# cvxgrp/cvxpygen

Hardware: AMD Instinct MI355X
Metric: QP instances solved/sec (batched MPC QP, OSQP; inputs resident in HBM) (higher is better)
Workload: dtype f64

## Files before the change

### cvxpygen_amd/codegen.py

```python

from __future__ import annotations

import os
import shutil
import subprocess
from typing import List, Optional, Sequence

import numpy as np

from .solve_program import GEN_EXTRA_SLOTS, LANES, RaggedProgram, execution_steps, padded_offsets_fit

CSRC = os.path.join(os.path.dirname(os.path.abspath(__file__)), 'csrc')


class ProgramTooLarge(Exception):
    """the family's solve program cannot be made LDS-resident: no specialised library for it"""


def emit_program_header(rp: RaggedProgram, name: str = 'family', plan=None, depth: int = 2, cross: int = 4,
                        pad_offsets: bool = False, group_offsets: int = 4, batch: int = 1, early: int = 4) -> str:
    out: List[str] = []
    w = out.append
    w(f'// Generated by cvxpygen_amd.codegen for problem family "{name}" -- do not edit.')
    w(f'// solve program: {rp.n_phases} phases, {rp.n_chunks} chunks, {int(rp.ctab[:, 0].sum())} steps, '
# ... 537 lines not shown
    if sync:
        for _ in plist:
            w('        cpgw::block_sync();')
    w('    } break;')
    w('    }')
    w('}')
    w('}  // namespace cpg')
    return '\n'.join(out) + '\n' + epilogue


def factor_fingerprint(fac) -> int:
    h = 0x811C9DC5
    ct = np.asarray(fac.ctab, dtype=np.int32).reshape(-1, 4)[:, [0, 1, 3]]
    for arr in (np.ascontiguousarray(ct), np.ascontiguousarray(fac.tlen, dtype=np.uint32)):
        for b in arr.tobytes():
            h = ((h ^ b) * 0x01000193) & 0xFFFFFFFF
    return h


FACTOR_LOOKAHEAD = int(os.environ.get('CPG_FACTOR_LOOKAHEAD', 3))
FACTOR_BY_LEVEL = os.environ.get('CPG_FACTOR_BY_LEVEL', '1') != '0'
FACTOR_LOOKAHEAD_CHUNKS = int(os.environ.get('CPG_FACTOR_LOOKAHEAD_CHUNKS', 3))
FACTOR_DUMMY_DOUBLES = 2


def factor_levels(ctab) -> List[List[int]]:
    ct = np.asarray(ctab, dtype=np.int64).reshape(-1, 4)
    levels, cur = [], []
    for c in range(ct.shape[0]):
        cur.append(c)
        if int(ct[c, 1]) & 1:
            levels.append(cur)
            cur = []
    if cur:
        levels.append(cur)
    return levels


def factor_chunk_kinds(fac, nnzL: int, N: int, inverse_from: Optional[int] = None) -> List[str]:
    ct = np.asarray(fac.ctab, dtype=np.int64).reshape(-1, 4)
    nch = ct.shape[0]
    task = np.asarray(fac.task, dtype=np.int64).reshape(nch, -1)
    inv0 = nch if inverse_from is None else int(inverse_from)
    kinds = []
    for c in range(nch):
        t = task[c][task[c] != 0xFFFFFFFF] & 0x7FFFFFFF
# ... 307 lines not shown
        return False
    per_wave = max(per_wave, fac + (fac & 1))
    return tab + 8 * 8 * per_wave <= LDS_BYTES


def instance_header(plan, out_dir: str, name: str = 'family') -> Optional[str]:
    from . import refactor_plan as _rp
    d = plan.desc
    o = plan.osqp_shared or plan.osqp
    Ps, As = o.pruned(d.P, d.A)
    rpl = _rp.shared_mode_plan(Ps, As, o)
    if not instance_program_fits(rpl):
        return None
    dims = dict(N=d.n_var, M=d.m, NEQ=d.n_eq)
    mg = rpl.merged
    if mg is None:
        prog, fac = rpl.sol, emit_factor_program(rpl.fac, rpl.nnzL, rpl.n + rpl.m, by_level=FACTOR_BY_LEVEL)
    else:
        import types
        dims['NNZX'] = mg.nnzX
        prog = mg.sol
        fac = emit_factor_program(types.SimpleNamespace(ctab=mg.f_ctab, tlen=mg.f_len, task=mg.f_task), rpl.nnzL, rpl.n + rpl.m,
                                  zero=mg.fac_len - 1, one=mg.one_pos, inverse_from=mg.base.fac.n_chunks, by_level=FACTOR_BY_LEVEL)
    return write_instance_header(prog, os.path.join(os.path.abspath(out_dir), f'cpg_instance_{name}.h'), name,
                                 row_programs=shared_row_programs(Ps, As), dims=dims, epilogue=fac, lean=True)


RESIDENT_MAX_REGS = int(os.environ.get('CPG_RESIDENT_MAX_REGS', 160))
RESIDENT_MAX_STEPS = int(os.environ.get('CPG_RESIDENT_MAX_STEPS', 320))
RESIDENT_ACC_BASE = int(os.environ.get('CPG_RESIDENT_ACC_BASE', 32))
RESIDENT_GATHER_BATCH = int(os.environ.get('CPG_RESIDENT_GATHER_BATCH', 12))
RESIDENT_ACC_PAIRS = int(os.environ.get('CPG_RESIDENT_ACC_PAIRS', 112))


def resident_compiler_flags(defs: Sequence[str]) -> List[str]:
    return []


def matrix_parameters(desc) -> bool:
    import scipy.sparse as _sps
    NP = desc.NP
    return any(_sps.csr_matrix(desc.maps[k])[:, :NP].nnz > 0 for k in ('P', 'A'))


def resident_program_fits(rpl, np_var: Optional[int] = None) -> bool:
    rp = rpl.sol
# ... 716 lines not shown
```

### cvxpygen_amd/csrc/cpg_hip.cpp

```cpp
#include "../../include/cpg_hip.h"

#include <math.h>
#include <stdio.h>
#include <stdlib.h>
#include <string.h>

#include <algorithm>
#include <string>
#include <type_traits>
#include <vector>

#include "cpg_osqp_kernel.h"
#include "cpg_osqp_refactor.h"
#include "cpg_osqp_resident.h"
#include "cpg_osqp_team.h"
#include "cpg_osqp_squad.h"
#include "cpg_clarabel_kernel.h"

#include <hip/hip_runtime.h>
typedef hipStream_t rt_stream_t;
typedef hipEvent_t rt_event_t;
#define RT_CHECK(expr)                                                                         \
    do {                                                                                       \
        hipError_t e_ = (expr);                                                                \
// ... 12 lines not shown
};
struct ResultBufs {
    DevBuf prim, dual, obj, pri, dua, iter, status;
    int ensure(size_t B, const cpg::DevFamily &F);
    void free();
    int copy_out(rt_stream_t stream, size_t first, size_t B, const cpg::DevFamily &F, double *prim_h, double *dual_h,
                 double *obj_h, double *pri_h, double *dua_h, int32_t *iter_h, int32_t *status_h) const;
};

struct cpg_solver_s {
    int device = 0;
    rt_stream_t stream{};
    rt_event_t ev0{}, ev1{};
    bool have_events = false;
    float last_ms = 0.f;
    std::vector<void *> owned;
    std::vector<void *> update_owned;
    cpg::DevFamily F{};
    cpg::DevUpdate U{};
    bool have_update = false;
    cpg::DevRefactor R{};
    bool refactor_mode = false;
    std::vector<void *> refactor_owned;
    cpg::DevResident Rs{};
    std::vector<void *> resident_owned;
    cpg::DevGradient Gd{};
    bool have_gradient = false;
    std::vector<void *> gradient_owned;
    DevBuf g_theta, g_x, g_y, g_dprim, g_dtheta;
    const int *gv_ptr = nullptr, *gv_src = nullptr;
    int n_gv = 0;
    std::vector<void *> gv_owned;
    rt_event_t ev_after{};
    cpg::DevSettings S{};
    int waves_per_block = 0, inst_per_wave = 1, blocks_per_cu = 0;
    int program_in_lds = -1;
    bool squad_ok = false;
    cpg::DevShRegs SRg{};
    bool sreg_ok = false;
    double sreg_rho = 0.0, sreg_sigma = 0.0;
    std::vector<void *> sreg_owned;
    std::vector<void *> ireg_owned;
    int num_cu = 256;
    size_t lds_limit = 160 * 1024;
    unsigned *d_counter = nullptr;
    int n_vary_x = 0, n_vary_z = 0;
// ... 1429 lines not shown
        else if (kind == CPG_K_SIGMA) fkc[d] = h->F.sigma;
        else if (kind == CPG_K_RHO) { if (idx < 0 || (size_t)idx >= m) return false; fkrow[d] = idx; }
        else if (kind != CPG_K_NONE) return false;
    }
    return true;
}

#ifdef CPG_GENI_HEADER
struct InstanceTables {
    int nnzX;
    int sol_chunks, sol_nnz, sol_slots;
    const int32_t *sol_ctab; const uint32_t *sol_desc; const uint16_t *sol_cols; const int32_t *sol_kind, *sol_idx;
    int fac_chunks, fac_triples;
    const int32_t *fac_ctab; const uint32_t *fac_task, *fac_len, *fac_a, *fac_b, *fac_k;
};

static int set_instance_executor(cpg_handle_t h, const cpg_osqp_refactor_t *r, const InstanceTables &g,
                                 const std::vector<double> &fkc, const std::vector<int> &fkrow) {
    std::vector<void *> &own = h->refactor_owned;
    cpg::DevRefactor &R = h->R;
    const size_t n = h->F.n, m = h->F.m, N = n + m;
    int rc = CPG_OK;
    R.gi_ok = 0;
    std::vector<unsigned short> gcols, grows, glcol;
    std::vector<unsigned> gsrc, gdk;
    std::vector<unsigned long long> gtri;
    std::vector<double> gkc;
#ifdef CPG_GENI_N
    const bool geni_dims = h->F.n == CPG_GENI_N && h->F.m == CPG_GENI_M && h->F.n_eq == CPG_GENI_NEQ;
#else
    const bool geni_dims = true;
#endif
#ifdef CPG_GENI_NNZX
    const bool merged_lib = true;
#else
    const bool merged_lib = false;
#endif
    if (!(geni_dims && (g.nnzX > 0) == merged_lib && g.sol_chunks == CPG_GENI_NCHUNKS && g.sol_nnz == CPG_GENI_NNZ && g.sol_slots == CPG_GENI_NSLOTS))
        return CPG_OK;
    const size_t nd = (size_t)r->nnzL + N, nx = (size_t)g.nnzX;
    const unsigned hsh = program_fingerprint(g.sol_ctab, g.sol_desc, g.sol_cols, g.sol_chunks, g.sol_nnz);
    static const int steps[][4] = CPG_GENI_STEPS;
    static const int chunk_shift[] = CPG_GENI_CHUNK_SHIFT;
    bool ok = hsh == CPG_GENI_FINGERPRINT;
    {
        const int nn[3] = {CPG_GENI_AROWS_N, CPG_GENI_PROWS_N, CPG_GENI_ATROWS_N};
        for (int k = 0; ok && k < 3; k++) {
            if ((int)h->rows_hdr[k].size() != 4 * nn[k]) ok = false;
// ... 7 lines not shown
        glcol.assign((size_t)CPG_GENI_NREGS * 64, (unsigned short)0);
        std::vector<char> taken((size_t)CPG_GENI_NREGS * 64, 0);
        for (int t = 0; ok && t < CPG_GENI_NSTEPS; t++) {
            const int e = steps[t][0], cnt = steps[t][1], reg = steps[t][2], sh = steps[t][3];
            if (reg < 0 || reg >= CPG_GENI_NREGS) { ok = false; break; }
            for (int l = 0; l < cnt; l++) {
                int kind = g.sol_kind[e + l], idx = g.sol_idx[e + l];
                if (kind == 4) {
                    if (idx < 0 || (size_t)idx >= nx) { ok = false; break; }
                    kind = 3; idx += (int)N;
                }
                if (kind < 0 || kind > 3 || idx < 0 || idx >= (1 << 28)) { ok = false; break; }
                const size_t at = (size_t)reg * 64 + (size_t)(l + sh);
                if (taken[at]) { ok = false; break; }
                taken[at] = 1;
                gsrc[at] = ((unsigned)kind << 28) | (unsigned)idx;
                if (kind == 2) {
                    if (idx >= r->nnzL || r->Lcol[idx] < 0 || r->Lcol[idx] > 0xFFFF) { ok = false; break; }
                    glcol[at] = (unsigned short)r->Lcol[idx];
                }
            }
        }
    }
#ifdef CPG_GENI_FAC_NSTEPS
    if (ok) {
        static const int fch[][3] = CPG_GENI_FAC_CHUNKS;
        const size_t fac_end = nx ? nd + nx + 2 : nd + 1;
        const size_t one = nd + nx;
        unsigned hsh2 = 0x811C9DC5u;
        auto mix = [&](unsigned v) { for (int k = 0; k < 4; k++) { hsh2 = (hsh2 ^ ((v >> (8 * k)) & 0xFFu)) * 0x01000193u; } };
        const unsigned idle_dst = CPG_GENI_FAC_DUMMY_DOUBLES ? (unsigned)fac_end : 0xFFFFu;
        ok = g.fac_chunks == CPG_GENI_FAC_NCHUNKS && fac_end - 1 == (size_t)CPG_GENI_FAC_ZERO && fac_end + CPG_GENI_FAC_DUMMY_DOUBLES <= 0xFFFFu;
#ifdef CPG_GENI_FAC_ONE
        ok = ok && one == (size_t)CPG_GENI_FAC_ONE;
#endif
        for (int c = 0; ok && c < g.fac_chunks; c++) { mix((unsigned)g.fac_ctab[4 * c]); mix((unsigned)g.fac_ctab[4 * c + 1]); mix((unsigned)g.fac_ctab[4 * c + 3]); }
        for (size_t e = 0; ok && e < (size_t)g.fac_chunks * 64; e++) mix(g.fac_len[e]);
        ok = ok && hsh2 == CPG_GENI_FAC_FINGERPRINT;
        if (ok) {
            const unsigned long long Z = (unsigned long long)(fac_end - 1);
            gtri.assign((size_t)CPG_GENI_FAC_NSTEPS * 64, Z | (Z << 16) | (Z << 32));
            gdk.assign((size_t)g.fac_chunks * 64, idle_dst);
            gkc.assign((size_t)g.fac_chunks * 64, 0.0);
            size_t step = 0;
            for (int c = 0; ok && c < g.fac_chunks; c++) {
                const int L = g.fac_ctab[4 * c];
// ... 22 lines not shown
                    const unsigned t = nx ? (t0 & 0x7FFFFFFFu) : t0;
                    if (t >= nd + nx) { ok = false; break; }
                    const int kr = t < nd ? fkrow[t] : -1;
                    gdk[(size_t)c * 64 + l] = t | ((unsigned)(kr + 1) << 16);
                    gkc[(size_t)c * 64 + l] = t < nd ? fkc[t] : 0.0;
                }
            }
            if (ok && step != (size_t)CPG_GENI_FAC_NSTEPS) ok = false;
        }
        if (ok) {
            if ((rc = upload<unsigned long long>(h, own, gtri.data(), gtri.size(), &R.gf_tri))) return rc;
            if ((rc = upload<unsigned>(h, own, gdk.data(), gdk.size(), &R.gf_dk))) return rc;
            if ((rc = upload<double>(h, own, gkc.data(), gkc.size(), &R.gf_kc))) return rc;
        }
    }
#else
    ok = ok && !nx;
#endif
    if (ok) {
        if ((rc = upload<unsigned short>(h, own, glcol.data(), glcol.size(), &R.gi_lcol))) return rc;
        if ((rc = upload<unsigned short>(h, own, gcols.data(), gcols.size(), &R.gi_cols))) return rc;
        if ((rc = upload<unsigned short>(h, own, grows.data(), grows.size(), &R.gi_rows))) return rc;
        if ((rc = upload<unsigned>(h, own, gsrc.data(), gsrc.size(), &R.gi_src))) return rc;
    }
    if ((rc = rt_sync(h))) return rc;
    R.gi_ok = ok ? 1 : 0;
    return CPG_OK;
}
#endif

int cpg_hip_set_refactor(cpg_handle_t h, const cpg_osqp_refactor_t *r) {
    if (h && h->conic) { set_error("not available for a conic (interior-point) handle"); return CPG_E_BADARG; }
    if (!h || !r) { set_error("null argument"); return CPG_E_BADARG; }
    int rc = rt_set_device(h->device);
    if (rc) return rc;
    if ((rc = rt_sync_linked(h))) return rc;
    free_list(h->refactor_owned);
    free_list(h->resident_owned); h->Rs = cpg::DevResident{};
    free_list(h->ireg_owned);
    std::vector<void *> &own = h->refactor_owned;
    cpg::DevRefactor &R = h->R;
    R.fam_cf = nullptr; R.fam_ct = nullptr; R.fam_rho = 0.0; R.fam_sigma = 0.0;
    const size_t n = h->F.n, m = h->F.m, N = n + m;
    R.nnzP = r->nnzP; R.nnzA = r->nnzA; R.nnzL = r->nnzL; R.n_eq = h->F.n_eq; R.np_var = r->np_var;
    R.scaling_iters = r->scaling_iters; R.d_base = r->d_base;
    R.fac_chunks = r->fac_chunks; R.sol_nnz = r->sol_nnz; R.sol_slots = r->sol_slots;
// ... 49 lines not shown
    if ((rc = upload_csr(h, own, r->map_q, &R.map_q))) return rc;
    if ((rc = upload_csr(h, own, r->map_u, &R.map_u))) return rc;
    if ((rc = upload_csr(h, own, r->map_d, &R.map_d))) return rc;
    R.buf_doubles = (long long)(r->nnzP + 2 * r->nnzA + 3 * n + 4 * m + r->nnzL + 2 * N + std::max(R.sol_nnz, R.gs_nnz) + 64);
    R.shared_mats = r->shared_mats ? 1 : 0; R.cs = 1.0;
    R.Ps = R.As = R.Ars = R.Ds = R.Dinvs = R.Es = R.Einvs = nullptr;
    std::vector<double> ars, dinv, einv;
    if (r->shared_mats) {
        if (!r->Ps || !r->As || !r->D || !r->E || !(r->c > 0.0)) { set_error("shared-matrix mode needs Ps, As, D, E, c"); return CPG_E_BADARG; }
        ars.resize((size_t)r->nnzA); dinv.resize(n); einv.resize(m);
        for (int k = 0; k < r->nnzA; k++) ars[k] = r->As[r->Aent[k]];
        for (size_t i = 0; i < n; i++) dinv[i] = 1.0 / r->D[i];
        for (size_t i = 0; i < m; i++) einv[i] = 1.0 / r->E[i];
        R.cs = r->c;
        if ((rc = upload<double>(h, own, r->Ps, (size_t)r->nnzP, &R.Ps))) return rc;
        if ((rc = upload<double>(h, own, r->As, (size_t)r->nnzA, &R.As))) return rc;
        if ((rc = upload<double>(h, own, ars.data(), ars.size(), &R.Ars))) return rc;
        if ((rc = upload<double>(h, own, r->D, n, &R.Ds))) return rc;
        if ((rc = upload<double>(h, own, dinv.data(), n, &R.Dinvs))) return rc;
        if ((rc = upload<double>(h, own, r->E, m, &R.Es))) return rc;
        if ((rc = upload<double>(h, own, einv.data(), m, &R.Einvs))) return rc;
    }
    R.gf_tri = nullptr; R.gf_dk = nullptr; R.gf_kc = nullptr;
    R.gi_ok = 0; R.gi_cols = R.gi_rows = nullptr; R.gi_src = nullptr; R.gi_lcol = nullptr; R.fac_kc = nullptr; R.fac_krow = nullptr; R.fac_kc_cl = nullptr; R.fac_krow_cl = nullptr; R.fac_kind_cl = nullptr; R.fac_idx_cl = nullptr;
    std::vector<double> fkc, fkc_cl;
    std::vector<int> fkrow, fkrow_cl;

    if (r->shared_mats) {
        if (!kkt_constants(h, r, fkc, fkrow)) { set_error("cpg_hip_set_refactor: KKT source table out of range"); return CPG_E_BADARG; }
        const size_t nd = (size_t)r->nnzL + N;
        fkc_cl.assign((size_t)r->fac_chunks * 64, 0.0); fkrow_cl.assign((size_t)r->fac_chunks * 64, -1);
        for (size_t e = 0; e < fkc_cl.size(); e++) {
            const unsigned t = r->fac_task[e];
            if (t == 0xFFFFFFFFu) continue;
            if (t >= nd) { set_error("cpg_hip_set_refactor: factorisation task out of range"); return CPG_E_BADARG; }
            fkc_cl[e] = fkc[t]; fkrow_cl[e] = fkrow[t];
        }
        if ((rc = upload<double>(h, own, fkc.data(), fkc.size(), &R.fac_kc))) return rc;
        if ((rc = upload<int>(h, own, fkrow.data(), fkrow.size(), &R.fac_krow))) return rc;
        if ((rc = upload<double>(h, own, fkc_cl.data(), fkc_cl.size(), &R.fac_kc_cl))) return rc;
        if ((rc = upload<int>(h, own, fkrow_cl.data(), fkrow_cl.size(), &R.fac_krow_cl))) return rc;
    }
#ifdef CPG_GENI_HEADER
    if (r->shared_mats) {
        const InstanceTables g{0, r->sol_chunks, r->sol_nnz, r->sol_slots, r->sol_ctab, r->sol_desc, r->sol_cols, r->sol_kind, r->sol_idx,
                               r->fac_chunks, r->fac_triples, r->fac_ctab, r->fac_task, r->fac_len, r->fac_a, r->fac_b, r->fac_k};
        if ((rc = set_instance_executor(h, r, g, fkc, fkrow))) return rc;
// ... 786 lines not shown
    *stream = (void *)h->stream;
    return CPG_OK;
}

int cpg_hip_get_instance_tables(cpg_handle_t h, uint16_t *cols, int32_t n_cols, uint16_t *rows, int32_t n_rows, int32_t *row_bytes) {
    if (!h || !cols || !rows || !row_bytes) { set_error("null argument"); return CPG_E_BADARG; }
#ifdef CPG_GENI_HEADER
    const int32_t nc = ((CPG_GENI_NSTEPS + 3) / 4) * 256, nr = ((CPG_GENI_NCHUNKS + 3) / 4) * 256;
    if (h->conic || !h->R.gi_ok || !h->R.gi_cols || !h->R.gi_rows) { set_error("cpg_hip_get_instance_tables: the handle does not run the generated instance executor"); return CPG_E_BADARG; }
    if (n_cols != nc || n_rows != nr) { set_error("cpg_hip_get_instance_tables: table sizes differ from the library's"); return CPG_E_BADARG; }
    int rc = rt_set_device(h->device);
    if (rc) return rc;
    if ((rc = rt_d2h(h, cols, h->R.gi_cols, (size_t)nc * sizeof(uint16_t)))) return rc;
    if ((rc = rt_d2h(h, rows, h->R.gi_rows, (size_t)nr * sizeof(uint16_t)))) return rc;
    *row_bytes = geni_row_bytes ? 1 : 0;
    return rt_sync(h);
#else
    (void)n_cols; (void)n_rows;
    set_error("cpg_hip_get_instance_tables: this library has no generated instance executor");
    return CPG_E_UNSUPPORTED;
#endif
}

int cpg_hip_last_kernel_ms(cpg_handle_t h, float *ms) {
    if (!h || !ms) { set_error("null argument"); return CPG_E_BADARG; }
    RT_CHECK(hipEventSynchronize(h->ev1));
    RT_CHECK(hipEventElapsedTime(ms, h->ev0, h->ev1));
    return CPG_OK;
}

int cpg_hip_solve_batch(cpg_handle_t h, int64_t B, const double *theta, double *prim, double *dual, double *obj,
                        int32_t *iter, int32_t *status, double *pri_res, double *dua_res) {
    return cpg_hip_solve_batch_state(h, B, theta, nullptr, nullptr, prim, dual, obj, iter, status, pri_res, dua_res);
}

int cpg_hip_solve_batch_state(cpg_handle_t h, int64_t B, const double *theta, const double *state_in, double *state_out,
                              double *prim, double *dual, double *obj, int32_t *iter, int32_t *status,
                              double *pri_res, double *dua_res) {
    int rc = check_solve_args(h, B, theta, prim, dual, obj, iter, status, pri_res, dua_res);
    if (rc || B == 0) return rc;
    if ((rc = rt_set_device(h->device))) return rc;
    const size_t b = (size_t)B, npv = (size_t)np_var(h);
    ResultBufs &out = h->s_out;
    if ((rc = ensure(h->s_theta, b * npv * sizeof(double))) || (rc = out.ensure(b, h->F))) return rc;
    if ((rc = rt_h2d(h, h->s_theta.p, theta, b * npv * sizeof(double)))) return rc;
    const size_t state_bytes = b * ((size_t)h->F.n + 2 * (size_t)h->F.m + 1) * sizeof(double);
// ... 120 lines not shown
```

### cvxpygen_amd/csrc/cpg_osqp_refactor.h

```cpp
#pragma once

#include "cpg_osqp_kernel.h"

#ifdef CPG_GENI_HEADER
#include CPG_GENI_HEADER
#endif
#ifdef CPG_GENI_FAC_BY_LEVEL
#define CPG_GENI_FAC_DUMMY_DOUBLES 2u
#else
#define CPG_GENI_FAC_DUMMY_DOUBLES 0u
#endif
#if defined(__HIP_DEVICE_COMPILE__)
#define CPG_REGION_MARK(s) asm volatile("; cpg-region " s)
#else
#define CPG_REGION_MARK(s) ((void)0)
#endif
#ifdef CPG_GENS_HEADER
#include CPG_GENS_HEADER
#define CPG_GENS_ACTIVE(geni, shared, crlds) (!(geni) && !(shared) && !(crlds))
#else
#define CPG_GENS_ACTIVE(geni, shared, crlds) false
#endif

namespace cpg {
// ... 20 lines not shown
    const int *Ap, *Ai, *Arp, *Aent, *Acol, *Pp, *Pi, *Prp, *Pent, *Pcol;
    const int *Lcol, *ksrc_kind, *ksrc_idx;
    const int *fac_ctab;
    const unsigned *fac_task, *fac_len, *fac_a, *fac_b, *fac_k;
    int fac_chunks;
    const int *sol_kind, *sol_idx;
    const unsigned short *sol_fpos;
    int sol_nnz, sol_slots;
    const unsigned *sol_stab;
    const unsigned *sol_cr;
    int sol_pairs;
    const double *P_base, *A_base, *q_base, *u_base;
    const double *q_setup;
    double d_base;
    DevCsr map_P, map_A, map_q, map_u, map_d;
    long long buf_doubles;
    int shared_mats;
    const double *Ps, *As, *Ars, *Ds, *Dinvs, *Es, *Einvs;
    double cs;
    int gi_ok;
    const unsigned short *gi_cols, *gi_rows;
    const unsigned *gi_src;
    const unsigned short *gi_lcol;
    const unsigned long long *gf_tri;
    const unsigned *gf_dk;
    const double *gf_kc;
    const unsigned short *gs_cols, *gs_rows;
    const int *gs_kind, *gs_idx;
    int gs_ok, gs_nnz;
    const double *fac_kc;
    const int *fac_krow;
    const double *fac_kc_cl;
    const int *fac_krow_cl;
    const int *fac_kind_cl, *fac_idx_cl;
    const double *fam_cf;
    const signed char *fam_ct;
    double fam_rho, fam_sigma;
};

#define CPG_K_NONE 0
#define CPG_K_P 1
#define CPG_K_A 2
#define CPG_K_SIGMA 3
#define CPG_K_RHO 4

CPG_DEV double lim_scaling(double v) { v = v < 1e-4 ? 1.0 : v; return v > 1e4 ? 1e4 : v; }
// ... 261 lines not shown
            const double v = (kc - kr) - acc;
            if (t0.task >= (unsigned)R.nnzL) cpgw::gst(Dil, t0.task - (unsigned)R.nnzL, 1.0 / v);
            else cpgw::gst(Ml, t0.task, v);
        }
        if (cpgw::read_first_lane(h0.last)) { if (LDS) cpgw::lds_order(); else cpgw::mem_order(); }
        h0 = h1; h1 = h2; t0 = t1; t1 = t2; i0 = i1;
    }
    if (LDS) cpgw::lds_order(); else cpgw::mem_order();
}

#ifdef CPG_GENI_HEADER
CPG_DEV void load_instance_coefficients(const DevRefactor &R, const double *Ml, const double *Dil, double (&cf)[CPG_GENI_NREGS], int lane) {
    const unsigned ln = (unsigned)cpgw::opaque(lane);
#pragma unroll
    for (int t = 0; t < CPG_GENI_NREGS; t++) {
        const unsigned code = cpgw::gld(R.gi_src, (unsigned)t * 64u + ln);
        const unsigned col = (unsigned)cpgw::opaque((int)cpgw::gld(R.gi_lcol, (unsigned)t * 64u + ln));
        const unsigned kind = code >> 28, idx = code & 0x0FFFFFFFu;
        const double a = kind == 3u ? Dil[idx] : Ml[kind == 2u ? idx : 0u], b = Dil[kind == 2u ? col : 0u];
        cf[t] = kind == 2u ? -(a * b) : (kind == 3u ? a : (kind == 1u ? 1.0 : 0.0));
    }
}

#ifdef CPG_GENI_NNZX
#ifndef CPG_SREG_LDS_REGS
#define CPG_SREG_LDS_REGS 20
#endif
struct SharedRegExec {
    static constexpr bool active = true;
    static constexpr int nslots = CPG_GENI_NSLOTS + CPG_GEN_EXTRA_SLOTS;
    static constexpr unsigned ncols = ((CPG_GENI_NSTEPS + 3u) / 4u) * 256u, nrows = ((CPG_GENI_NCHUNKS + 3u) / 4u) * 256u;
    static constexpr int nlds = CPG_SREG_LDS_REGS < CPG_GENI_NREGS ? CPG_SREG_LDS_REGS : CPG_GENI_NREGS;
    static constexpr int nreg = CPG_GENI_NREGS - nlds;
    const double *gcf;
    const unsigned short *gcols, *grows, *lc = nullptr, *lr = nullptr;
    const double *lcf = nullptr;
    double cf[nreg > 0 ? nreg : 1];
    CPG_DEV explicit SharedRegExec(const DevShRegs &t) : gcf(t.cf), gcols(t.cols), grows(t.rows) {}
    CPG_DEV size_t stage(double *lds) {
        unsigned short *c = (unsigned short *)lds, *r = c + ncols;
        double *v = lds + (ncols + nrows) / 4u;
        const unsigned t0 = cpgw::thread_in_block(), nt = cpgw::block_threads();
        for (unsigned t = t0; t < ncols; t += nt) c[t] = cpgw::gld(gcols, t);
        for (unsigned t = t0; t < nrows; t += nt) r[t] = cpgw::gld(grows, t);
        for (unsigned t = t0; t < 64u * (unsigned)nlds; t += nt) v[t] = cpgw::gld(gcf, 64u * (unsigned)nreg + t);
        lc = c; lr = r; lcf = v;
// ... 259 lines not shown
                substitution_values<true>(R, B, lane);
            } else {
                numeric_ldl(R, B, F0.sigma, lane);
                substitution_values<false, GENS>(R, B, lane);
            }
        };
#ifdef CPG_GENI_HEADER
        auto factor_in_lds = [&]() __attribute__((always_inline)) {
            cpgw::mem_order();
#ifdef CPG_GENI_FAC_NSTEPS
            if (lane == 0) w[CPG_GENI_FAC_ZERO] = 0.0;
#ifdef CPG_GENI_FAC_ONE
            if (lane == 0) w[CPG_GENI_FAC_ONE] = 1.0;
#endif
            cpgw::lds_order();
            CPG_REGION_MARK("factor begin");
            numeric_ldl_gen(R.gf_tri, R.gf_dk, R.gf_kc, (const double *)B.rinv, w, lane);
            CPG_REGION_MARK("factor end");
#else
            numeric_ldl_m<true>(R, w, w + R.nnzL, (const double *)B.rinv, lane);
#endif
            CPG_INST_PROBE_SPLIT();
            CPG_REGION_MARK("coefficients begin");
            load_instance_coefficients(R, w, w + R.nnzL, cf, lane);
            CPG_REGION_MARK("coefficients end");
            cpgw::lds_order();
            CPG_INST_PROBE_SPLIT();
            for (unsigned t = (unsigned)lane; t < (unsigned)ldw; t += 64u) w[t] = 0.0;
            for (unsigned i = (unsigned)lane; i < n; i += 64u) qs[i] = cpgw::gld((const double *)B.q, i);
            for (unsigned i = (unsigned)lane; i < m; i += 64u) us[i] = cpgw::gld((const double *)B.u, i);
            cpgw::lds_order();
        };
        if (__builtin_expect(S.debug_stage == 2, 0)) { if (lane == 0) { Bt.status[b] = 11; Bt.iter[b] = 0; } continue; }
        CPG_INST_PROBE();
        if (GENI) {
            bool other = false;
#pragma unroll
            for (int s = 0; s < NSZ; s++) other = other || ((unsigned)lane + 64u * (unsigned)s < m && ct[s] != fct[s]);
            if (fam_start && cpgw::ballot(other) == 0ull) {
                const unsigned ln = (unsigned)cpgw::opaque(lane);
#pragma unroll
                for (int t = 0; t < CPG_GENI_NREGS; t++) cf[t] = cpgw::gld(R.fam_cf, (unsigned)t * 64u + ln);
                for (unsigned t = (unsigned)lane; t < (unsigned)ldw; t += 64u) w[t] = 0.0;
#pragma unroll
                for (int s = 0; s < NSX; s++) { const unsigned i = (unsigned)lane + 64u * (unsigned)s; if (i < n) qs[i] = qv[GENI ? s : 0]; }
#pragma unroll
                for (int s = 0; s < NSZ; s++) { const unsigned i = (unsigned)lane + 64u * (unsigned)s; if (i < m) us[i] = uv[GENI ? s : 0]; }
// ... 311 lines not shown
```

### cvxpygen_amd/runtime.py

```python

from __future__ import annotations

import ctypes as C
import os
import time
from dataclasses import dataclass, field
from typing import Dict, List, Optional, Sequence

import numpy as np
import scipy.sparse as sp

from . import osqp_setup as _setup
from . import solve_program as _sp
from .canon_builder import canon_lu
from .descriptor import CPG_INF, FamilyDescriptor

_dp = C.POINTER(C.c_double)
_ip = C.POINTER(C.c_int32)
_u16p = C.POINTER(C.c_uint16)
_i8p = C.POINTER(C.c_int8)

STATUS_STRINGS = {1: 'solved', 2: 'solved inaccurate', 3: 'primal infeasible',
                  4: 'primal infeasible inaccurate', 5: 'dual infeasible',
                  6: 'dual infeasible inaccurate', 7: 'maximum iterations reached',
# ... 67 lines not shown
                ('sol_kind', _ip), ('sol_idx', _ip), ('sol_lcol', _ip),
                ('rows_A', _RowsProgram), ('rows_P', _RowsProgram), ('rows_At', _RowsProgram),
                ('out_ax', C.c_int32), ('out_px', C.c_int32), ('out_aty', C.c_int32)]


class _Gradient(C.Structure):
    _fields_ = [('NP', C.c_int32), ('Pcolidx', _ip), ('Acolidx', _ip), ('tptr', _ip), ('tkind', _ip),
                ('tidx', _ip), ('tcoef', _dp)]


class _Update(C.Structure):
    _fields_ = [('np_var', C.c_int32), ('q_base', _dp), ('u_base', _dp), ('d_base', C.c_double),
                ('map_q', _Csr), ('map_u', _Csr), ('map_d', _Csr)]


def default_lib_path() -> str:
    return os.path.join(os.path.dirname(os.path.abspath(__file__)), 'csrc', 'libcpg_hip.so')


class CpgLibrary:

    SYMBOLS = ['cpg_hip_device_count', 'cpg_hip_create_osqp', 'cpg_hip_create_clarabel', 'cpg_hip_destroy', 'cpg_hip_last_error',
               'cpg_hip_status_string', 'cpg_hip_set_default_settings', 'cpg_hip_set_setting',
               'cpg_hip_get_setting', 'cpg_hip_set_build_option', 'cpg_hip_set_handover', 'cpg_hip_last_phase_ms', 'cpg_hip_set_update', 'cpg_hip_set_refactor', 'cpg_hip_set_refactor_merged', 'cpg_hip_set_shared_registers', 'cpg_hip_set_instance_registers', 'cpg_hip_get_instance_tables', 'cpg_hip_set_resident', 'cpg_hip_set_gradient', 'cpg_hip_gradient_batch',
               'cpg_hip_set_gradient_vars', 'cpg_hip_gradient_batch_device',
               'cpg_hip_solve_batch',
               'cpg_hip_solve_batch_device', 'cpg_hip_solve_batch_state', 'cpg_hip_solve_batch_device_state', 'cpg_hip_solve_batches_pipelined', 'cpg_hip_host_malloc',
               'cpg_hip_host_free', 'cpg_hip_synchronize', 'cpg_hip_get_stream', 'cpg_hip_last_kernel_ms',
               'cpg_hip_set_launch', 'cpg_hip_set_program_placement', 'cpg_hip_malloc', 'cpg_hip_free', 'cpg_hip_memcpy_h2d',
               'cpg_hip_memcpy_d2h']

    def __init__(self, path: Optional[str] = None):
        path = path or default_lib_path()
        if not os.path.exists(path):
            raise RuntimeError(
                f'HIP extension {path} not found: build it with `python -m cvxpygen_amd.csrc.build` '
                '(there is no CPU fallback)')
        self.path = path
        L = C.CDLL(path)
        self.L = L
        L.cpg_hip_last_error.restype = C.c_char_p
        L.cpg_hip_status_string.restype = C.c_char_p
        L.cpg_hip_status_string.argtypes = [C.c_int32]
        L.cpg_hip_device_count.argtypes = [_ip]
        L.cpg_hip_create_osqp.argtypes = [C.POINTER(_Family), C.c_int, C.POINTER(C.c_void_p)]
        L.cpg_hip_destroy.argtypes = [C.c_void_p]
        L.cpg_hip_set_default_settings.argtypes = [C.c_void_p]
        L.cpg_hip_set_setting.argtypes = [C.c_void_p, C.c_char_p, C.c_double]
        L.cpg_hip_get_setting.argtypes = [C.c_void_p, C.c_char_p, _dp]
        L.cpg_hip_set_build_option.argtypes = [C.c_void_p, C.c_char_p, C.c_double]
        L.cpg_hip_set_handover.argtypes = [C.c_void_p, C.c_void_p]
        L.cpg_hip_last_phase_ms.argtypes = [C.c_void_p, C.POINTER(C.c_float), C.POINTER(C.c_float), C.POINTER(C.c_int64)]
        L.cpg_hip_set_update.argtypes = [C.c_void_p, C.POINTER(_Update)]
        L.cpg_hip_set_refactor.argtypes = [C.c_void_p, C.POINTER(_Refactor)]
        L.cpg_hip_set_resident.argtypes = [C.c_void_p, C.POINTER(_Refactor), C.POINTER(_Resident)]
        L.cpg_hip_set_refactor_merged.argtypes = [C.c_void_p, C.POINTER(_Refactor), C.POINTER(_Resident)]
        L.cpg_hip_get_instance_tables.argtypes = [C.c_void_p, _u16p, C.c_int32, _u16p, C.c_int32, C.POINTER(C.c_int32)]
        L.cpg_hip_set_shared_registers.argtypes = [C.c_void_p, C.POINTER(_Resident), _dp, C.c_int32, C.c_double, C.c_double]
        L.cpg_hip_set_instance_registers.argtypes = [C.c_void_p, C.POINTER(_Resident), _dp, C.c_int32, _i8p, C.c_double, C.c_double]
        L.cpg_hip_set_gradient.argtypes = [C.c_void_p, C.POINTER(_Gradient)]
        L.cpg_hip_gradient_batch.argtypes = [C.c_void_p, C.c_int64, _dp, _dp, _dp, _dp, _dp]
        L.cpg_hip_set_gradient_vars.argtypes = [C.c_void_p, C.c_int32, _ip]
        L.cpg_hip_gradient_batch_device.argtypes = [C.c_void_p, C.c_int64] + [C.c_void_p] * 6
        L.cpg_hip_solve_batch.argtypes = [C.c_void_p, C.c_int64, _dp, _dp, _dp, _dp, _ip, _ip, _dp, _dp]
        L.cpg_hip_solve_batch_device.argtypes = [C.c_void_p, C.c_int64] + [C.c_void_p] * 8
        L.cpg_hip_solve_batch_state.argtypes = [C.c_void_p, C.c_int64, _dp, _dp, _dp, _dp, _dp, _dp, _ip, _ip, _dp, _dp]
        L.cpg_hip_solve_batch_device_state.argtypes = [C.c_void_p, C.c_int64] + [C.c_void_p] * 10
        L.cpg_hip_synchronize.argtypes = [C.c_void_p]
        L.cpg_hip_solve_batches_pipelined.argtypes = [C.c_void_p, C.c_int64, C.c_int32, _dp, _dp, _dp, _dp, _ip, _ip, _dp, _dp]
        L.cpg_hip_host_malloc.argtypes = [C.c_void_p, C.c_size_t, C.POINTER(C.c_void_p)]
        L.cpg_hip_host_free.argtypes = [C.c_void_p, C.c_void_p]
        L.cpg_hip_get_stream.argtypes = [C.c_void_p, C.POINTER(C.c_void_p)]
        L.cpg_hip_last_kernel_ms.argtypes = [C.c_void_p, C.POINTER(C.c_float)]
        L.cpg_hip_set_launch.argtypes = [C.c_void_p, C.c_int, C.c_int, C.c_int]
        L.cpg_hip_set_program_placement.argtypes = [C.c_void_p, C.c_int]
        L.cpg_hip_malloc.argtypes = [C.c_void_p, C.c_size_t, C.POINTER(C.c_void_p)]
        L.cpg_hip_free.argtypes = [C.c_void_p, C.c_void_p]
        L.cpg_hip_memcpy_h2d.argtypes = [C.c_void_p, C.c_void_p, C.c_void_p, C.c_size_t]
        L.cpg_hip_memcpy_d2h.argtypes = [C.c_void_p, C.c_void_p, C.c_void_p, C.c_size_t]

# ... 1187 lines not shown
```

### include/cpg_hip.h

```cpp
#ifndef CPG_HIP_H
#define CPG_HIP_H

#include <stddef.h>
#include <stdint.h>

#ifdef __cplusplus
extern "C" {
#endif

#define CPG_OK 0
#define CPG_E_BADARG (-1)
#define CPG_E_HIP (-2)
#define CPG_E_NOMEM (-3)
#define CPG_E_UNSUPPORTED (-4)

#define CPG_STATUS_SOLVED 1
#define CPG_STATUS_SOLVED_INACCURATE 2
#define CPG_STATUS_PRIMAL_INFEASIBLE 3
#define CPG_STATUS_PRIMAL_INFEASIBLE_INACCURATE 4
#define CPG_STATUS_DUAL_INFEASIBLE 5
#define CPG_STATUS_DUAL_INFEASIBLE_INACCURATE 6
#define CPG_STATUS_MAX_ITER_REACHED 7
#define CPG_STATUS_NON_CVX 9
#define CPG_STATUS_UNSOLVED 11
// ... 149 lines not shown
const char *cpg_hip_status_string(int32_t status);

int cpg_hip_set_default_settings(cpg_handle_t h);
int cpg_hip_set_setting(cpg_handle_t h, const char *name, double value);
int cpg_hip_get_setting(cpg_handle_t h, const char *name, double *value);
int cpg_hip_set_build_option(cpg_handle_t h, const char *name, double value);
int cpg_hip_set_handover(cpg_handle_t h, cpg_handle_t per_instance);
int cpg_hip_last_phase_ms(cpg_handle_t h, float *ms_shared, float *ms_per_instance, int64_t *n_handed_over);

int cpg_hip_set_update(cpg_handle_t h, const cpg_osqp_update_t *upd);

int cpg_hip_set_refactor(cpg_handle_t h, const cpg_osqp_refactor_t *rf);

int cpg_hip_set_refactor_merged(cpg_handle_t h, const cpg_osqp_refactor_t *rf, const cpg_osqp_resident_t *mg);

int cpg_hip_set_shared_registers(cpg_handle_t h, const cpg_osqp_resident_t *mg, const double *coef, int32_t n_coef,
                                 double rho, double sigma);

int cpg_hip_set_instance_registers(cpg_handle_t h, const cpg_osqp_resident_t *mg, const double *coef, int32_t n_coef,
                                   const int8_t *row_class, double rho, double sigma);

int cpg_hip_get_instance_tables(cpg_handle_t h, uint16_t *cols, int32_t n_cols, uint16_t *rows, int32_t n_rows, int32_t *row_bytes);

int cpg_hip_set_resident(cpg_handle_t h, const cpg_osqp_refactor_t *rf, const cpg_osqp_resident_t *rs);

int cpg_hip_set_gradient(cpg_handle_t h, const cpg_osqp_gradient_t *g);
int cpg_hip_gradient_batch(cpg_handle_t h, int64_t B, const double *theta_var, const double *sol_x,
                           const double *sol_y, const double *dx, double *dtheta);
int cpg_hip_set_gradient_vars(cpg_handle_t h, int32_t n_gv, const int32_t *idx);
int cpg_hip_gradient_batch_device(cpg_handle_t h, int64_t B, const double *d_theta_var, const double *d_sol_x,
                                  const double *d_sol_y, const double *d_dvars, double *d_dtheta, cpg_handle_t after);

int cpg_hip_solve_batch(cpg_handle_t h, int64_t B, const double *theta_var, double *prim, double *dual,
                        double *obj, int32_t *iter, int32_t *status, double *pri_res, double *dua_res);

int cpg_hip_solve_batch_device(cpg_handle_t h, int64_t B, const double *d_theta_var, double *d_prim,
                               double *d_dual, double *d_obj, int32_t *d_iter, int32_t *d_status,
                               double *d_pri_res, double *d_dua_res);
int cpg_hip_solve_batch_state(cpg_handle_t h, int64_t B, const double *theta_var, const double *state_in,
                              double *state_out, double *prim, double *dual, double *obj, int32_t *iter,
                              int32_t *status, double *pri_res, double *dua_res);
int cpg_hip_solve_batch_device_state(cpg_handle_t h, int64_t B, const double *d_theta_var, const double *d_state_in,
                                     double *d_state_out, double *d_prim, double *d_dual, double *d_obj,
                                     int32_t *d_iter, int32_t *d_status, double *d_pri_res, double *d_dua_res);
int cpg_hip_solve_batches_pipelined(cpg_handle_t h, int64_t B, int32_t n_batches, const double *theta_var,
                                    double *prim, double *dual, double *obj, int32_t *iter, int32_t *status,
// ... 19 lines not shown
```

Baseline: 6.306 million.

## Gather instance coefficients in two passes: scale L entries in LDS, then offset-load

Replaces per-register coefficient loading with a two-pass scheme. First, each referenced L entry is negated and scaled by its column diagonal in place in LDS, using a precomputed scale table. Then every register coefficient is read through a precomputed byte-offset table. The aim is to drop per-register kind decoding and repeated multiplies in the coefficient extraction step, at the cost of extra device tables, extra host-side validation, and an LDS ordering barrier between the passes. A debug accessor for the new tables is also added.

```diff
diff --git a/cvxpygen_amd/codegen.py b/cvxpygen_amd/codegen.py
--- a/cvxpygen_amd/codegen.py
+++ b/cvxpygen_amd/codegen.py
@@ -583,6 +583,20 @@
 FACTOR_BY_LEVEL = os.environ.get('CPG_FACTOR_BY_LEVEL', '1') != '0'
 FACTOR_LOOKAHEAD_CHUNKS = int(os.environ.get('CPG_FACTOR_LOOKAHEAD_CHUNKS', 3))
 FACTOR_DUMMY_DOUBLES = 2
+COEFFICIENT_TWO_PASS = os.environ.get('CPG_COEFFICIENT_TWO_PASS', '1') != '0'
+COEFFICIENT_SCALE_BATCH = int(os.environ.get('CPG_COEFFICIENT_SCALE_BATCH', 7))
+COEFFICIENT_OFFSET_BATCH = int(os.environ.get('CPG_COEFFICIENT_OFFSET_BATCH', 0))
+
+
+def coefficient_scale_rounds(prog, sol_kind, sol_idx) -> int:
+    from .solve_program import execution_steps
+    from .refactor_plan import SRC_NEG_L
+    kind, idx = np.asarray(sol_kind), np.asarray(sol_idx)
+    seen = set()
+    for _, _, e, cnt in execution_steps(prog):
+        k = np.arange(e, e + cnt)
+        seen.update(int(i) for i in idx[k][kind[k] == SRC_NEG_L])
+    return -(-len(seen) // 64)
 
 
 def factor_levels(ctab) -> List[List[int]]:
@@ -936,6 +950,13 @@
         prog = mg.sol
         fac = emit_factor_program(types.SimpleNamespace(ctab=mg.f_ctab, tlen=mg.f_len, task=mg.f_task), rpl.nnzL, rpl.n + rpl.m,
                                   zero=mg.fac_len - 1, one=mg.one_pos, inverse_from=mg.base.fac.n_chunks, by_level=FACTOR_BY_LEVEL)
+        if COEFFICIENT_TWO_PASS and FACTOR_BY_LEVEL and 8 * (mg.fac_len + FACTOR_DUMMY_DOUBLES) <= 0xFFFF:
+            rounds = coefficient_scale_rounds(prog, mg.sol_kind, mg.sol_idx)
+            fac += f'#define CPG_GENI_COEF_TWO_PASS 1\n#define CPG_GENI_COEF_SCALE_ROUNDS {rounds}\n'
+            if COEFFICIENT_SCALE_BATCH > 0:
+                fac += f'#define CPG_COEF_SCALE_BATCH {COEFFICIENT_SCALE_BATCH}\n'
+            if COEFFICIENT_OFFSET_BATCH > 0:
+                fac += f'#define CPG_COEF_OFFSET_BATCH {COEFFICIENT_OFFSET_BATCH}\n'
     return write_instance_header(prog, os.path.join(os.path.abspath(out_dir), f'cpg_instance_{name}.h'), name,
                                  row_programs=shared_row_programs(Ps, As), dims=dims, epilogue=fac, lean=True)
 
diff --git a/cvxpygen_amd/csrc/cpg_hip.cpp b/cvxpygen_amd/csrc/cpg_hip.cpp
--- a/cvxpygen_amd/csrc/cpg_hip.cpp
+++ b/cvxpygen_amd/csrc/cpg_hip.cpp
@@ -58,6 +58,7 @@
     cpg::DevRefactor R{};
     bool refactor_mode = false;
     std::vector<void *> refactor_owned;
+    int coef_scale_entries = 0;
     cpg::DevResident Rs{};
     std::vector<void *> resident_owned;
     cpg::DevGradient Gd{};
@@ -1533,8 +1534,8 @@
     const size_t n = h->F.n, m = h->F.m, N = n + m;
     int rc = CPG_OK;
     R.gi_ok = 0;
-    std::vector<unsigned short> gcols, grows, glcol;
-    std::vector<unsigned> gsrc, gdk;
+    std::vector<unsigned short> gcols, grows, glcol, goff;
+    std::vector<unsigned> gsrc, gdk, gscale;
     std::vector<unsigned long long> gtri;
     std::vector<double> gkc;
 #ifdef CPG_GENI_N
@@ -1588,6 +1589,28 @@
             }
         }
     }
+#ifdef CPG_COEF_TWO_PASS_ACTIVE
+    if (ok) {
+        const size_t zero = (size_t)CPG_GENI_FAC_ZERO, one = (size_t)CPG_GENI_FAC_ONE, dummy = zero + 1;
+        ok = CPG_GENI_FAC_DUMMY_DOUBLES >= 1u && nd + nx == one && one + 1 == zero && 8 * (zero + 1 + CPG_GENI_FAC_DUMMY_DOUBLES) <= 0xFFFFu;
+        std::vector<char> scaled(ok ? (size_t)r->nnzL : 0, 0);
+        goff.assign((size_t)CPG_GENI_NREGS * 64, (unsigned short)(8 * zero));
+        for (size_t at = 0; ok && at < gsrc.size(); at++) {
+            const unsigned kind = gsrc[at] >> 28, idx = gsrc[at] & 0x0FFFFFFFu;
+            size_t pos = zero;
+            if (kind == 1) pos = one;
+            else if (kind == 2) { pos = idx; scaled[idx] = 1; }
+            else if (kind == 3) { pos = (size_t)r->nnzL + idx; if (idx >= N + nx) ok = false; }
+            goff[at] = (unsigned short)(8 * pos);
+        }
+        for (size_t e = 0; ok && e < scaled.size(); e++)
+            if (scaled[e]) gscale.push_back((unsigned)e | (((unsigned)r->nnzL + (unsigned)r->Lcol[e]) << 16));
+        for (size_t k = 0; ok && k < gscale.size(); k++) if ((gscale[k] >> 16) >= nd) ok = false;
+        ok = ok && (gscale.size() + 63) / 64 == (size_t)CPG_GENI_COEF_SCALE_ROUNDS;
+        h->coef_scale_entries = ok ? (int)gscale.size() : 0;
+        if (ok) gscale.resize((size_t)(CPG_GENI_COEF_SCALE_ROUNDS > 0 ? CPG_GENI_COEF_SCALE_ROUNDS : 1) * 64, (unsigned)dummy | ((unsigned)zero << 16));
+    }
+#endif
 #ifdef CPG_GENI_FAC_NSTEPS
     if (ok) {
         static const int fch[][3] = CPG_GENI_FAC_CHUNKS;
@@ -1656,6 +1679,10 @@
         if ((rc = upload<unsigned short>(h, own, gcols.data(), gcols.size(), &R.gi_cols))) return rc;
         if ((rc = upload<unsigned short>(h, own, grows.data(), grows.size(), &R.gi_rows))) return rc;
         if ((rc = upload<unsigned>(h, own, gsrc.data(), gsrc.size(), &R.gi_src))) return rc;
+#ifdef CPG_COEF_TWO_PASS_ACTIVE
+        if ((rc = upload<unsigned>(h, own, gscale.data(), gscale.size(), &R.gi_scale))) return rc;
+        if ((rc = upload<unsigned short>(h, own, goff.data(), goff.size(), &R.gi_off))) return rc;
+#endif
     }
     if ((rc = rt_sync(h))) return rc;
     R.gi_ok = ok ? 1 : 0;
@@ -1751,7 +1778,7 @@
         if ((rc = upload<double>(h, own, einv.data(), m, &R.Einvs))) return rc;
     }
     R.gf_tri = nullptr; R.gf_dk = nullptr; R.gf_kc = nullptr;
-    R.gi_ok = 0; R.gi_cols = R.gi_rows = nullptr; R.gi_src = nullptr; R.gi_lcol = nullptr; R.fac_kc = nullptr; R.fac_krow = nullptr; R.fac_kc_cl = nullptr; R.fac_krow_cl = nullptr; R.fac_kind_cl = nullptr; R.fac_idx_cl = nullptr;
+    R.gi_ok = 0; R.gi_cols = R.gi_rows = nullptr; R.gi_src = nullptr; R.gi_lcol = nullptr; R.gi_scale = nullptr; R.gi_off = nullptr; R.fac_kc = nullptr; R.fac_krow = nullptr; R.fac_kc_cl = nullptr; R.fac_krow_cl = nullptr; R.fac_kind_cl = nullptr; R.fac_idx_cl = nullptr;
     std::vector<double> fkc, fkc_cl;
     std::vector<int> fkrow, fkrow_cl;
 
@@ -2584,6 +2611,25 @@
 #endif
 }
 
+int cpg_hip_get_coefficient_tables(cpg_handle_t h, uint32_t *scale, int32_t n_scale, uint16_t *offsets, int32_t n_offsets, int32_t *n_entries) {
+    if (!h || !scale || !offsets || !n_entries) { set_error("null argument"); return CPG_E_BADARG; }
+#ifdef CPG_COEF_TWO_PASS_ACTIVE
+    const int32_t ns = (CPG_GENI_COEF_SCALE_ROUNDS > 0 ? CPG_GENI_COEF_SCALE_ROUNDS : 1) * 64, no = CPG_GENI_NREGS * 64;
+    if (h->conic || !h->R.gi_ok || !h->R.gi_scale || !h->R.gi_off) { set_error("cpg_hip_get_coefficient_tables: the handle does not run the generated instance executor"); return CPG_E_BADARG; }
+    if (n_scale != ns || n_offsets != no) { set_error("cpg_hip_get_coefficient_tables: table sizes differ from the library's"); return CPG_E_BADARG; }
+    int rc = rt_set_device(h->device);
+    if (rc) return rc;
+    if ((rc = rt_d2h(h, scale, h->R.gi_scale, (size_t)ns * sizeof(uint32_t)))) return rc;
+    if ((rc = rt_d2h(h, offsets, h->R.gi_off, (size_t)no * sizeof(uint16_t)))) return rc;
+    *n_entries = h->coef_scale_entries;
+    return rt_sync(h);
+#else
+    (void)n_scale; (void)n_offsets;
+    set_error("cpg_hip_get_coefficient_tables: this library extracts the instance coefficients register by register");
+    return CPG_E_UNSUPPORTED;
+#endif
+}
+
 int cpg_hip_last_kernel_ms(cpg_handle_t h, float *ms) {
     if (!h || !ms) { set_error("null argument"); return CPG_E_BADARG; }
     RT_CHECK(hipEventSynchronize(h->ev1));
diff --git a/cvxpygen_amd/csrc/cpg_osqp_refactor.h b/cvxpygen_amd/csrc/cpg_osqp_refactor.h
--- a/cvxpygen_amd/csrc/cpg_osqp_refactor.h
+++ b/cvxpygen_amd/csrc/cpg_osqp_refactor.h
@@ -66,6 +66,8 @@
     const unsigned short *gi_cols, *gi_rows;
     const unsigned *gi_src;
     const unsigned short *gi_lcol;
+    const unsigned *gi_scale;
+    const unsigned short *gi_off;
     const unsigned long long *gf_tri;
     const unsigned *gf_dk;
     const double *gf_kc;
@@ -373,6 +375,50 @@
     }
 }
 
+#if defined(CPG_GENI_COEF_TWO_PASS) && defined(CPG_GENI_FAC_BY_LEVEL) && defined(CPG_GENI_FAC_ONE)
+#define CPG_COEF_TWO_PASS_ACTIVE 1
+#ifndef CPG_COEF_SCALE_BATCH
+#define CPG_COEF_SCALE_BATCH CPG_GENI_COEF_SCALE_ROUNDS
+#endif
+#ifndef CPG_COEF_OFFSET_BATCH
+#define CPG_COEF_OFFSET_BATCH CPG_GENI_NREGS
+#endif
+CPG_DEV void gather_instance_coefficients(const DevRefactor &R, double *w, double (&cf)[CPG_GENI_NREGS], int lane) {
+    constexpr int NR = CPG_GENI_COEF_SCALE_ROUNDS, NB = CPG_COEF_SCALE_BATCH < NR ? CPG_COEF_SCALE_BATCH : NR;
+    const unsigned ln = (unsigned)cpgw::opaque(lane);
+    constexpr int NA = NB > 0 ? NB : 1;
+    unsigned sw[NA];
+#pragma unroll
+    for (int t = 0; t < NB; t++) sw[t] = cpgw::gld(R.gi_scale, (unsigned)t * 64u + ln);
+#pragma unroll
+    for (int r0 = 0; r0 < NR; r0 += NB) {
+        double a[NA], d[NA];
+        unsigned nx[NA];
+#pragma unroll
+        for (int t = 0; t < NB; t++) if (r0 + t < NR) { a[t] = w[sw[t] & 0xFFFFu]; d[t] = w[sw[t] >> 16]; }
+#pragma unroll
+        for (int t = 0; t < NB; t++) if (r0 + NB + t < NR) nx[t] = cpgw::gld(R.gi_scale, (unsigned)(r0 + NB + t) * 64u + ln);
+        cpgw::sched_fence();
+#pragma unroll
+        for (int t = 0; t < NB; t++) if (r0 + t < NR) w[sw[t] & 0xFFFFu] = -(a[t] * d[t]);
+        cpgw::sched_fence();
+#pragma unroll
+        for (int t = 0; t < NB; t++) if (r0 + NB + t < NR) sw[t] = nx[t];
+    }
+    cpgw::lds_order();
+    constexpr int OB = CPG_COEF_OFFSET_BATCH < CPG_GENI_NREGS ? CPG_COEF_OFFSET_BATCH : CPG_GENI_NREGS;
+#pragma unroll
+    for (int t0 = 0; t0 < CPG_GENI_NREGS; t0 += OB) {
+        unsigned short off[OB];
+#pragma unroll
+        for (int t = 0; t < OB; t++) if (t0 + t < CPG_GENI_NREGS) off[t] = cpgw::gld(R.gi_off, (unsigned)(t0 + t) * 64u + ln);
+#pragma unroll
+        for (int t = 0; t < OB; t++) if (t0 + t < CPG_GENI_NREGS) cf[t0 + t] = *(const double *)((const char *)w + off[t]);
+        if (OB < CPG_GENI_NREGS) cpgw::sched_fence();
+    }
+}
+#endif
+
 #ifdef CPG_GENI_NNZX
 #ifndef CPG_SREG_LDS_REGS
 #define CPG_SREG_LDS_REGS 20
@@ -678,7 +724,11 @@
 #endif
             CPG_INST_PROBE_SPLIT();
             CPG_REGION_MARK("coefficients begin");
+#ifdef CPG_COEF_TWO_PASS_ACTIVE
+            gather_instance_coefficients(R, w, cf, lane);
+#else
             load_instance_coefficients(R, w, w + R.nnzL, cf, lane);
+#endif
             CPG_REGION_MARK("coefficients end");
             cpgw::lds_order();
             CPG_INST_PROBE_SPLIT();
diff --git a/cvxpygen_amd/runtime.py b/cvxpygen_amd/runtime.py
--- a/cvxpygen_amd/runtime.py
+++ b/cvxpygen_amd/runtime.py
@@ -113,7 +113,7 @@
 
     SYMBOLS = ['cpg_hip_device_count', 'cpg_hip_create_osqp', 'cpg_hip_create_clarabel', 'cpg_hip_destroy', 'cpg_hip_last_error',
                'cpg_hip_status_string', 'cpg_hip_set_default_settings', 'cpg_hip_set_setting',
-               'cpg_hip_get_setting', 'cpg_hip_set_build_option', 'cpg_hip_set_handover', 'cpg_hip_last_phase_ms', 'cpg_hip_set_update', 'cpg_hip_set_refactor', 'cpg_hip_set_refactor_merged', 'cpg_hip_set_shared_registers', 'cpg_hip_set_instance_registers', 'cpg_hip_get_instance_tables', 'cpg_hip_set_resident', 'cpg_hip_set_gradient', 'cpg_hip_gradient_batch',
+               'cpg_hip_get_setting', 'cpg_hip_set_build_option', 'cpg_hip_set_handover', 'cpg_hip_last_phase_ms', 'cpg_hip_set_update', 'cpg_hip_set_refactor', 'cpg_hip_set_refactor_merged', 'cpg_hip_set_shared_registers', 'cpg_hip_set_instance_registers', 'cpg_hip_get_instance_tables', 'cpg_hip_get_coefficient_tables', 'cpg_hip_set_resident', 'cpg_hip_set_gradient', 'cpg_hip_gradient_batch',
                'cpg_hip_set_gradient_vars', 'cpg_hip_gradient_batch_device',
                'cpg_hip_solve_batch',
                'cpg_hip_solve_batch_device', 'cpg_hip_solve_batch_state', 'cpg_hip_solve_batch_device_state', 'cpg_hip_solve_batches_pipelined', 'cpg_hip_host_malloc',
@@ -147,6 +147,7 @@
         L.cpg_hip_set_resident.argtypes = [C.c_void_p, C.POINTER(_Refactor), C.POINTER(_Resident)]
         L.cpg_hip_set_refactor_merged.argtypes = [C.c_void_p, C.POINTER(_Refactor), C.POINTER(_Resident)]
         L.cpg_hip_get_instance_tables.argtypes = [C.c_void_p, _u16p, C.c_int32, _u16p, C.c_int32, C.POINTER(C.c_int32)]
+        L.cpg_hip_get_coefficient_tables.argtypes = [C.c_void_p, C.POINTER(C.c_uint32), C.c_int32, _u16p, C.c_int32, C.POINTER(C.c_int32)]
         L.cpg_hip_set_shared_registers.argtypes = [C.c_void_p, C.POINTER(_Resident), _dp, C.c_int32, C.c_double, C.c_double]
         L.cpg_hip_set_instance_registers.argtypes = [C.c_void_p, C.POINTER(_Resident), _dp, C.c_int32, _i8p, C.c_double, C.c_double]
         L.cpg_hip_set_gradient.argtypes = [C.c_void_p, C.POINTER(_Gradient)]
diff --git a/include/cpg_hip.h b/include/cpg_hip.h
--- a/include/cpg_hip.h
+++ b/include/cpg_hip.h
@@ -195,6 +195,8 @@
 
 int cpg_hip_get_instance_tables(cpg_handle_t h, uint16_t *cols, int32_t n_cols, uint16_t *rows, int32_t n_rows, int32_t *row_bytes);
 
+int cpg_hip_get_coefficient_tables(cpg_handle_t h, uint32_t *scale, int32_t n_scale, uint16_t *offsets, int32_t n_offsets, int32_t *n_entries);
+
 int cpg_hip_set_resident(cpg_handle_t h, const cpg_osqp_refactor_t *rf, const cpg_osqp_resident_t *rs);
 
 int cpg_hip_set_gradient(cpg_handle_t h, const cpg_osqp_gradient_t *g);
```

New measurement: 6.590 million (median of 6 runs). 1.04x the previous value.
